# joyecnu/STTODE

Measured on AMD Instinct MI355X. Metric: predicted-trajectories/sec (20-sample best-of-K), higher is better.
Workload: dtype f32

## Files before the change

### profiles/exp_chain_stamps.py

```python
import ctypes, os, sys
import numpy as np, torch
ROOT = os.path.dirname(os.path.dirname(os.path.abspath(__file__)))
sys.path.insert(0, ROOT); sys.path.insert(0, os.path.join(ROOT, 'tests'))
from helpers import make_args
from sttode_amd import STTODENet, capi, scenes
from sttode_amd.weights import make_weights, to_torch_state_dict
dev = torch.device('cuda:0')
m = STTODENet(make_args('eth', 8, 12), dev).eval()
m.load_state_dict(to_torch_state_dict(make_weights(1234)), strict=True)
L = capi.lib()
for S in [int(a) for a in sys.argv[1:]] or [128]:
    sb = scenes.make_scene_batch(range(S), 'eth')
    m.set_scene_batch(sb.past, sb.future, sb.scene_ptr)
    m.native().set_chain(1)
    for _ in range(3):
        m.inference(None)
    ngroups = (sb.n_agents * 20 + 127) // 128
    nwg = max(512, ngroups + (sb.n_agents + 15) // 16)
    dbg = torch.zeros(nwg * 4 * 16, dtype=torch.int64, device=dev)
    L.sttode_chain_debug_buffer.argtypes = [ctypes.c_void_p]
    L.sttode_chain_debug_buffer(dbg.data_ptr())
    m.inference(None)
    torch.cuda.synchronize()
    L.sttode_chain_debug_buffer(None)
    d = dbg.cpu().numpy().reshape(nwg, 4, 8, 2)
    valid = d[:, :, 0, 0] > 0
    cyc = d[..., 0].astype(np.float64); ns = d[..., 1].astype(np.float64) * 10.0
    names = ['mlp0x', 'mlp0y', 'gru', 'mlp1']
    print(f'scenes {S}: {ngroups} groups, {int(valid.sum())} stamped group passes')
    for k in range(4):
        dc = (cyc[:, :, k + 1] - cyc[:, :, k])[valid]; dn = (ns[:, :, k + 1] - ns[:, :, k])[valid]
        print(f'  {names[k]:6s} cycles median {np.median(dc):10.0f} min {dc.min():10.0f} max {dc.max():10.0f} | us median {np.median(dn) / 1e3:8.1f}  -> clock {np.median(dc) / np.median(dn):.2f} GHz')
    tot = (ns[:, :, 4] - ns[:, :, 0])[valid]
    t0 = ns[:, 0, 0][valid[:, 0]]
    print(f'  group total us median {np.median(tot) / 1e3:.1f} min {tot.min() / 1e3:.1f} max {tot.max() / 1e3:.1f}; first-group start spread {(t0.max() - t0.min()) / 1e3:.1f} us; '
          f'kernel span {(ns[:, :, 4][valid].max() - t0.min()) / 1e3:.1f} us')
    b3 = os.environ.get('STTODE_BF16X3', '0') not in ('', '0')
    per_tile = 12 * 32 if b3 else 16 * 64
    ideal = {'mlp0x': 152 * per_tile, 'mlp0y': 152 * per_tile, 'gru': 8 * 37 * per_tile, 'mlp1': 200 * per_tile}
    print('  MFMA-only cycles per phase (' + ('bf16x3' if b3 else 'f32') + '):', ideal)
```

### sttode_amd/csrc/chain.hpp

```cpp
#pragma once
#include <hip/hip_runtime.h>

typedef float f32x4 __attribute__((ext_vector_type(4)));

#define STT_WAVE 64
#define STT_FENCE() asm volatile("" ::: "memory")

__device__ __forceinline__ f32x4 mfma_k16(f32x4 acc, const f32x4 w, const f32x4 b) {
    acc = __builtin_amdgcn_mfma_f32_16x16x4f32(w[0], b[0], acc, 0, 0, 0);
    acc = __builtin_amdgcn_mfma_f32_16x16x4f32(w[1], b[1], acc, 0, 0, 0);
    acc = __builtin_amdgcn_mfma_f32_16x16x4f32(w[2], b[2], acc, 0, 0, 0);
    acc = __builtin_amdgcn_mfma_f32_16x16x4f32(w[3], b[3], acc, 0, 0, 0);
    return acc;
}

__device__ __forceinline__ f32x4 ld4(const float* p) { return *reinterpret_cast<const f32x4*>(p); }
__device__ __forceinline__ void st4(float* p, const f32x4 v) { *reinterpret_cast<f32x4*>(p) = v; }

__device__ __forceinline__ f32x4 relu4(f32x4 v) {
    v[0] = fmaxf(v[0], 0.f); v[1] = fmaxf(v[1], 0.f); v[2] = fmaxf(v[2], 0.f); v[3] = fmaxf(v[3], 0.f);
    return v;
}

__device__ __forceinline__ float sigmoidf_(float x) {
// ... 15 lines not shown

__device__ __forceinline__ void layernorm64(f32x4 (&x)[4], const float* __restrict__ gamma, const float* __restrict__ beta, int q) {
    float s = 0.f;
#pragma unroll
    for (int T = 0; T < 4; ++T) s += (x[T][0] + x[T][1]) + (x[T][2] + x[T][3]);
    const float mean = colsum_q(s) * (1.0f / 64.0f);
    float v = 0.f;
#pragma unroll
    for (int T = 0; T < 4; ++T)
#pragma unroll
        for (int r = 0; r < 4; ++r) { const float d = x[T][r] - mean; v += d * d; }
    const float rstd = 1.0f / sqrtf(colsum_q(v) * (1.0f / 64.0f) + 1e-5f);
#pragma unroll
    for (int T = 0; T < 4; ++T) {
        const f32x4 g = ld4(gamma + 16 * T + 4 * q), b = ld4(beta + 16 * T + 4 * q);
#pragma unroll
        for (int r = 0; r < 4; ++r) x[T][r] = (x[T][r] - mean) * rstd * g[r] + b[r];
    }
}

__device__ __forceinline__ void lds_barrier() { asm volatile("s_waitcnt lgkmcnt(0)\n\ts_barrier" ::: "memory"); }

__device__ __forceinline__ unsigned lds_addr(const void* p) {
    return (unsigned)(size_t)(const __attribute__((address_space(3))) void*)p;
}
__device__ __forceinline__ void glds16_asm(const void* gsrc, unsigned lds_dst) {
    unsigned keep;
    asm volatile("s_mov_b32 %0, m0\n\ts_mov_b32 m0, %2\n\ts_nop 0\n\tglobal_load_lds_dwordx4 %1, off\n\ts_mov_b32 m0, %0"
                 : "=&s"(keep) : "v"(gsrc), "s"(lds_dst) : "memory");
}
template <int OFS>
__device__ __forceinline__ void glds16_sv(const void* sbase, unsigned voff, unsigned lds_dst) {
    static_assert(OFS >= -4096 && OFS <= 4095, "global_load_lds_dwordx4: the immediate offset is 13-bit signed");
    unsigned keep;
    asm volatile("s_mov_b32 %0, m0\n\ts_mov_b32 m0, %3\n\ts_nop 0\n\tglobal_load_lds_dwordx4 %1, %2 offset:%4\n\ts_mov_b32 m0, %0"
                 : "=&s"(keep) : "v"(voff), "s"(sbase), "s"(lds_dst - (unsigned)OFS), "i"(OFS) : "memory");
}
```

### sttode_amd/csrc/chain32.hip

```cpp
#include "chain.hpp"
#include "latency_bodies.hpp"
#include "frontend_body.hpp"
#include "api_util.hpp"
#include "../../include/sttode_hip.h"
#include <cstdlib>
#include <cstddef>

#ifdef C32_DIAG_TRACE
__shared__ long long g_tr_ph[4];
#define C32_TRACE_BEGIN() long long _tr_t0 = 0, _tr_c0 = 0; if (threadIdx.x == 0 && A.dbg) { _tr_t0 = __builtin_amdgcn_s_memrealtime(); _tr_c0 = __builtin_amdgcn_s_memtime(); }
#define C32_TRACE_END(kind) do { if (threadIdx.x == 0 && A.dbg) { \
        const long long _t1 = __builtin_amdgcn_s_memrealtime(); unsigned _hw, _xcc; \
        asm volatile("s_getreg_b32 %0, hwreg(HW_REG_HW_ID)" : "=s"(_hw)); asm volatile("s_getreg_b32 %0, hwreg(HW_REG_XCC_ID)" : "=s"(_xcc)); \
        const unsigned long long _r = atomicAdd((unsigned long long*)A.dbg, 1ull); if ((long long)_r >= A.dbg[1]) break;  \
        long long* _p = A.dbg + 8 + _r * 12; _p[0] = A.trace_tag; _p[1] = blockIdx.x; _p[2] = (kind); _p[3] = _tr_t0; _p[4] = _t1; _p[5] = _hw; _p[6] = _xcc; \
        _p[8] = g_tr_ph[0]; _p[9] = g_tr_ph[1]; _p[10] = g_tr_ph[2]; _p[7] = __builtin_amdgcn_s_memtime() - _tr_c0; _p[11] = g_tr_ph[3]; } } while (0)
#define C32_TRACE_PHASE(i) do { if (threadIdx.x == 0) g_tr_ph[i] = __builtin_amdgcn_s_memrealtime(); } while (0)
#else
#define C32_TRACE_PHASE(i) do { } while (0)
#define C32_TRACE_BEGIN() do { } while (0)
#define C32_TRACE_END(kind) do { } while (0)
#endif

#include "role_body.hpp"
// ... 49 lines not shown
    int xcd_map;
    RoleArgs R;
    Role32Args R32;
};

template <int NY> struct C32Const {
    static constexpr int b2x = 0, b3x = 256, b2y = 288, b3y = 544, gb = 544 + 32 * NY, cb = gb + 384, b2m = cb + 32,
                         b3m = b2m + 256, total = b3m + 32 * NY;
};

__device__ __forceinline__ f32x16 splat16(float v) {
    f32x16 r;
#pragma unroll
    for (int e = 0; e < 16; ++e) r[e] = v;
    return r;
}
__device__ __forceinline__ f32x16 relu16(f32x16 v) {
#pragma unroll
    for (int e = 0; e < 16; ++e) v[e] = fmaxf(v[e], 0.f);
    return v;
}
__device__ __forceinline__ f32x16 ldrows(const float* p, int h) {
    f32x16 r;
#pragma unroll
    for (int a = 0; a < 4; ++a) {
        const f32x4 v = ld4(p + 8 * a + 4 * h);
        r[4 * a + 0] = v[0]; r[4 * a + 1] = v[1]; r[4 * a + 2] = v[2]; r[4 * a + 3] = v[3];
    }
    return r;
}

typedef const __attribute__((address_space(4))) int KProg;

template <int BUF, bool GEN>
struct ChainStreamT {
    static constexpr int kBuf = BUF;
    const char* pool; KProg* prog; f32x4* ring;
    unsigned ring_addr, loff;
    int len, p, par, lane, wave;
    int2 nxt_v;
    int cnt;
    __device__ __forceinline__ int2 entry(int q) const { return make_int2(prog[2 * q], prog[2 * q + 1]); }
    __device__ __forceinline__ void dma(int2 ev, int buf) {
        const char* src = pool + (size_t)ev.x * (GEN ? 16 : C32_TILE * 16) + wave * 1024;
        const int pieces = GEN ? ev.y : 4 * ev.y;
        const unsigned dst = __builtin_amdgcn_readfirstlane(ring_addr + (unsigned)buf * (BUF * 16) + (unsigned)wave * 1024);
#ifndef C32_DIAG_NODMA
#pragma unroll
        for (int i = 0; i < (BUF / 64 + 3) / 4; ++i)
            if (4 * i + wave < pieces) glds16_sv<0>(src + i * 4096, loff, dst + i * 4096);
#endif
    }
    __device__ __forceinline__ void init(const f32x4* pool_, const int2* prog_, int len_, f32x4* ring_) {
        pool = reinterpret_cast<const char*>(pool_); prog = (KProg*)prog_; len = len_; ring = ring_;
        ring_addr = lds_addr(ring_);
        lane = threadIdx.x & 63;
        loff = (unsigned)lane * 16;
        wave = __builtin_amdgcn_readfirstlane(threadIdx.x >> 6);
        p = 0; par = 0;
        const int2 e0 = entry(0);
        cnt = e0.y;
        dma(e0, 0);
        nxt_v = entry(1 % len);
    }
    __device__ __forceinline__ void begin() {
        __builtin_amdgcn_sched_barrier(0);
        cnt = nxt_v.y;
        dma(nxt_v, par ^ 1);
        int q = p + 2;
        q = q >= len ? q - len : q;
        nxt_v = entry(q);
        __builtin_amdgcn_sched_barrier(0);
    }
    __device__ __forceinline__ const f32x4* cur() const { return ring + par * BUF + lane; }
    __device__ __forceinline__ void end() {
        __builtin_amdgcn_sched_barrier(0);
#ifndef C32_DIAG_NOBARRIER
        asm volatile("s_waitcnt vmcnt(0)" ::: "memory");
        __syncthreads();
#endif
        p = p + 1 >= len ? 0 : p + 1;
        par ^= 1;
        __builtin_amdgcn_sched_barrier(0);
    }
};
typedef ChainStreamT<C32_CMAX * C32_TILE, false> ChainStream;

__device__ __forceinline__ void tile_mma(f32x16& acc, const f32x4* __restrict__ t, const f32x16& B) {
#pragma unroll
    for (int g = 0; g < 4; ++g) {
        const f32x4 a = t[g * 64];
#pragma unroll
        for (int r = 0; r < 4; ++r) acc = __builtin_amdgcn_mfma_f32_32x32x2f32(a[r], B[4 * g + r], acc, 0, 0, 0);
    }
}

__device__ __forceinline__ void gather_rows(const void* base, unsigned voff, unsigned slot_addr) {
    glds16_sv<0>(base, voff, slot_addr);
    glds16_sv<32>(base, voff, slot_addr + 1024);
    glds16_sv<64>(base, voff, slot_addr + 2048);
    glds16_sv<96>(base, voff, slot_addr + 3072);
}
__device__ __forceinline__ unsigned row_off(int row, int width, int h) { return (unsigned)row * (unsigned)(width * 4) + (unsigned)h * 16; }

struct Frag { f32x4 a[4]; };
__device__ __forceinline__ void ldfrag(Frag& f, const f32x4* __restrict__ t) {
#pragma unroll
    for (int g = 0; g < 4; ++g) f.a[g] = t[g * 64];
}
__device__ __forceinline__ void tile_mma2(f32x16& acc, const Frag& cur, const f32x16& B, Frag& nxt, const f32x4* __restrict__ tn) {
#pragma unroll
    for (int g = 0; g < 4; ++g) {
        if (g == 2 && tn) {
            ldfrag(nxt, tn);
            __builtin_amdgcn_sched_barrier(0);
        }
#pragma unroll
        for (int r = 0; r < 4; ++r) acc = __builtin_amdgcn_mfma_f32_32x32x2f32(cur.a[g][r], B[4 * g + r], acc, 0, 0, 0);
    }
}

template <int KH, class ST>
__device__ __forceinline__ void mlp_l12(ST& st, const f32x4* slot, const f32x4* zslot, const f32x16* Bh, const float* tab, unsigned aoff,
                                        const float* tab_next, unsigned aoff_next, f32x16 (&acc2)[8], int lane) {
    const unsigned slot_addr = __builtin_amdgcn_readfirstlane(lds_addr(slot));
    constexpr int KT1 = 1 + KH;
    static_assert((KT1 + 8) % 3 == 0, "hidden tile must be a whole number of chunks");
#pragma unroll
    for (int R = 0; R < 8; ++R) acc2[R] = splat16(0.f);
#pragma unroll 1
    for (int ht = 0; ht < 16; ++ht) {
        f32x16 h1, zb;
#pragma unroll
        for (int a = 0; a < 4; ++a) {
            const f32x4 v = slot[a * 64 + lane];
            h1[4 * a + 0] = v[0]; h1[4 * a + 1] = v[1]; h1[4 * a + 2] = v[2]; h1[4 * a + 3] = v[3];
        }
#pragma unroll
        for (int a = 0; a < 4; ++a) {
            const f32x4 v = zslot[a * 64 + lane];
            zb[4 * a + 0] = v[0]; zb[4 * a + 1] = v[1]; zb[4 * a + 2] = v[2]; zb[4 * a + 3] = v[3];
        }
        asm volatile("s_waitcnt lgkmcnt(0)" ::: "memory");
        __builtin_amdgcn_sched_barrier(0);
        const bool nl = ht + 1 < 16;
        const void* nb = nl ? (const void*)(reinterpret_cast<const char*>(tab) + 128 * (ht + 1)) : (const void*)tab_next;
        const unsigned no = nl ? aoff : aoff_next;
        Frag fr[2];
#pragma unroll
        for (int i = 0; i < KT1 + 8; ++i) {
            if (i % 3 == 0) {
                if (i > 0) st.end();
                ldfrag(fr[i & 1], st.cur());
                st.begin();
                if (i == 0) {
#ifndef C32_DIAG_NOGATHER
                    gather_rows(nb, no, slot_addr);
#endif
                    __builtin_amdgcn_sched_barrier(0);
                }
            }
            const f32x4* tn = (i % 3 < 2) ? st.cur() + (i % 3 + 1) * C32_TILE : nullptr;
            if (i == 0) {
                tile_mma2(h1, fr[i & 1], zb, fr[(i + 1) & 1], tn);
            } else if (i < KT1) {
                tile_mma2(h1, fr[i & 1], Bh[i - 1], fr[(i + 1) & 1], tn);
            } else {
                if (i == KT1) h1 = relu16(h1);
                tile_mma2(acc2[i - KT1], fr[i & 1], h1, fr[(i + 1) & 1], tn);
            }
        }
        st.end();
    }
}

template <int NO, class ST>
__device__ __forceinline__ void mlp_l3(ST& st, f32x16 (&acc2)[8], const float* __restrict__ b2, const float* __restrict__ b3,
                                       f32x16 (&out)[NO], int h) {
#pragma unroll
    for (int R = 0; R < 8; ++R) {
        STT_FENCE();
        const f32x16 b = ldrows(b2 + 32 * R, h);
        acc2[R] = relu16(acc2[R] + b);
        asm volatile("" : "+v"(acc2[R]));
    }
    STT_FENCE();
#pragma unroll
    for (int o = 0; o < NO; ++o) out[o] = ldrows(b3 + 32 * o, h);
    Frag fr[2];
#pragma unroll
    for (int i = 0; i < 8 * NO; ++i) {
        if (i % 3 == 0) {
            if (i > 0) st.end();
            ldfrag(fr[i & 1], st.cur());
            st.begin();
        }
        const f32x4* tn = (i % 3 < 2 && i + 1 < 8 * NO) ? st.cur() + (i % 3 + 1) * C32_TILE : nullptr;
        tile_mma2(out[i / 8], fr[i & 1], acc2[i % 8], fr[(i + 1) & 1], tn);
    }
    st.end();
}

typedef __bf16 bf16x8 __attribute__((ext_vector_type(8)));
typedef __bf16 bf16x2 __attribute__((ext_vector_type(2)));
typedef float f32x2v __attribute__((ext_vector_type(2)));
typedef unsigned u32x4v __attribute__((ext_vector_type(4)));
#define C32_TILE_B3 384
#define C32_BUF_B3 (C32_CMAX * C32_TILE_B3)
struct B3 { bf16x8 p[3][2]; };
__device__ __forceinline__ float bf_lo(unsigned u) { return __uint_as_float(u << 16); }
__device__ __forceinline__ float bf_hi(unsigned u) { return __uint_as_float(u & 0xffff0000u); }
__device__ __forceinline__ void split3(const f32x16& x, B3& o) {
#pragma unroll
    for (int kb = 0; kb < 2; ++kb) {
        unsigned hi[4], mi[4], lo[4];
#pragma unroll
        for (int q = 0; q < 4; ++q) {
            const float x0 = x[8 * kb + 2 * q], x1 = x[8 * kb + 2 * q + 1];
            const f32x2v v = {x0, x1};
            hi[q] = __builtin_bit_cast(unsigned, __builtin_convertvector(v, bf16x2));
            const float r0 = x0 - bf_lo(hi[q]), r1 = x1 - bf_hi(hi[q]);
            const f32x2v rv = {r0, r1};
            mi[q] = __builtin_bit_cast(unsigned, __builtin_convertvector(rv, bf16x2));
            const f32x2v qv = {r0 - bf_lo(mi[q]), r1 - bf_hi(mi[q])};
            lo[q] = __builtin_bit_cast(unsigned, __builtin_convertvector(qv, bf16x2));
        }
        const u32x4v H = {hi[0], hi[1], hi[2], hi[3]}, M = {mi[0], mi[1], mi[2], mi[3]}, L = {lo[0], lo[1], lo[2], lo[3]};
        o.p[0][kb] = __builtin_bit_cast(bf16x8, H);
        o.p[1][kb] = __builtin_bit_cast(bf16x8, M);
        o.p[2][kb] = __builtin_bit_cast(bf16x8, L);
    }
// ... 178 lines not shown
            tile_mma_b3n(az, st.cur() + T, hB[2]);
#pragma unroll
            for (int r = 0; r < 16; ++r) az[r] = C32_SIG(az[r]);
            STT_FENCE();
            f32x16 an = ldrows(gb + 3 * 96 + 32 * j, h);
            tile_mma_b3n(an, st.cur() + 2 * T, hB[0]);
            st.end(); st.begin();
            tile_mma_b3n(an, st.cur(), hB[1]);
            tile_mma_b3n(an, st.cur() + T, hB[2]);
            {
                const f32x16 bi = ldrows(gb + 2 * 96 + 32 * j, h);
#pragma unroll
                for (int r = 0; r < 16; ++r) an[r] = fmaf(ar[r], an[r], bi[r]);
            }
            STT_FENCE();
            tile_mma_b3n(an, st.cur() + 2 * T, eB);
            st.end();
            const f32x16 hp = b3_to_f32(hB[j]);
#pragma unroll
            for (int r = 0; r < 16; ++r) {
                const float ng = C32_TANH(an[r]);
                hn[j][r] = fmaf(az[r], hp[r] - ng, ng);
            }
        }
#pragma unroll
        for (int j = 0; j < 3; ++j) {
            hs[j] = hn[j];
            split3(hn[j], hB[j]);
        }
    }
}

template <bool ZS, class ST>
__device__ __forceinline__ f32x16 gru32_conv(ST& st, const float* cb, const f32x16& d, int t, int Tp, int h) {
    f32x16 e = ldrows(cb, h);
    Frag fa, fb;
    if (ZS) {
        const int k0 = 2 * t - 2, k1 = 2 * t + 3;
        const int g0 = (k0 > 0 ? k0 : 0) >> 3, g1 = (k1 < 2 * Tp - 1 ? k1 : 2 * Tp - 1) >> 3;
        const f32x4* tc = st.cur();
#pragma unroll
        for (int g = 0; g < 4; ++g)
            if (g >= g0 && g <= g1) fa.a[g] = tc[g * 64];
        st.begin();
#pragma unroll
        for (int g = 0; g < 4; ++g)
            if (g >= g0 && g <= g1)
#pragma unroll
                for (int r = 0; r < 4; ++r) e = __builtin_amdgcn_mfma_f32_32x32x2f32(fa.a[g][r], d[4 * g + r], e, 0, 0, 0);
    } else {
        ldfrag(fa, st.cur());
        st.begin();
        tile_mma2(e, fa, d, fb, nullptr);
    }
    e = relu16(e);
    st.end();
    return e;
}

template <bool ZS, class ST>
__device__ __forceinline__ void gru32_steps(ST& st, const float* gb, const float* cb, const f32x16& d, f32x16 (&hs)[3], int Tp, int h) {
    if (ZS) {
        const f32x16 e = gru32_conv<ZS>(st, cb, d, 0, Tp, h);
        Frag fa, fb;
#pragma unroll
        for (int j = 0; j < 3; ++j) {
            STT_FENCE();
            f32x16 ar = ldrows(gb + 0 * 96 + 32 * j, h);
            ldfrag(fa, st.cur()); st.begin();
            tile_mma2(ar, fa, e, fb, nullptr);
            st.end(); ldfrag(fa, st.cur() + 1 * C32_TILE); st.begin();
#pragma unroll
            for (int r = 0; r < 16; ++r) ar[r] = C32_SIG(ar[r]);
            STT_FENCE();
            f32x16 az = ldrows(gb + 1 * 96 + 32 * j, h);
            tile_mma2(az, fa, e, fb, nullptr);
            st.end(); st.begin();
#pragma unroll
            for (int r = 0; r < 16; ++r) az[r] = C32_SIG(az[r]);
            STT_FENCE();
            f32x16 an = ldrows(gb + 3 * 96 + 32 * j, h);
            {
                const f32x16 bi = ldrows(gb + 2 * 96 + 32 * j, h);
#pragma unroll
                for (int r = 0; r < 16; ++r) an[r] = fmaf(ar[r], an[r], bi[r]);
            }
            st.end(); ldfrag(fa, st.cur() + 2 * C32_TILE); st.begin();
            STT_FENCE();
            tile_mma2(an, fa, e, fb, nullptr);
            st.end();
#pragma unroll
            for (int r = 0; r < 16; ++r) {
                const float ng = C32_TANH(an[r]);
                hs[j][r] = fmaf(az[r], 0.f - ng, ng);
            }
        }
    }
#pragma unroll 1
    for (int t = ZS ? 1 : 0; t < Tp; ++t) {
        const f32x16 e = gru32_conv<ZS>(st, cb, d, t, Tp, h);
        Frag fa, fb;
        f32x16 hn[3];
#pragma unroll
        for (int j = 0; j < 3; ++j) {
            STT_FENCE();
            f32x16 ar = ldrows(gb + 0 * 96 + 32 * j, h);
            ldfrag(fa, st.cur()); st.begin();
            tile_mma2(ar, fa, e, fb, st.cur() + 1 * C32_TILE);
            tile_mma2(ar, fb, hs[0], fa, st.cur() + 2 * C32_TILE);
            tile_mma2(ar, fa, hs[1], fb, nullptr);
            st.end(); ldfrag(fa, st.cur()); st.begin();
            tile_mma2(ar, fa, hs[2], fb, st.cur() + 1 * C32_TILE);
#pragma unroll
            for (int r = 0; r < 16; ++r) ar[r] = C32_SIG(ar[r]);
            STT_FENCE();
            f32x16 az = ldrows(gb + 1 * 96 + 32 * j, h);
            tile_mma2(az, fb, e, fa, st.cur() + 2 * C32_TILE);
            tile_mma2(az, fa, hs[0], fb, nullptr);
            st.end(); ldfrag(fa, st.cur()); st.begin();
            tile_mma2(az, fa, hs[1], fb, st.cur() + 1 * C32_TILE);
            tile_mma2(az, fb, hs[2], fa, st.cur() + 2 * C32_TILE);
#pragma unroll
            for (int r = 0; r < 16; ++r) az[r] = C32_SIG(az[r]);
            STT_FENCE();
            f32x16 an = ldrows(gb + 3 * 96 + 32 * j, h);
            tile_mma2(an, fa, hs[0], fb, nullptr);
            st.end(); ldfrag(fa, st.cur()); st.begin();
            tile_mma2(an, fa, hs[1], fb, st.cur() + 1 * C32_TILE);
            tile_mma2(an, fb, hs[2], fa, st.cur() + 2 * C32_TILE);
            {
                const f32x16 bi = ldrows(gb + 2 * 96 + 32 * j, h);
#pragma unroll
                for (int r = 0; r < 16; ++r) an[r] = fmaf(ar[r], an[r], bi[r]);
            }
            STT_FENCE();
            tile_mma2(an, fa, e, fb, nullptr);
            st.end();
#pragma unroll
            for (int r = 0; r < 16; ++r) {
                const float ng = C32_TANH(an[r]);
                hn[j][r] = fmaf(az[r], hs[j][r] - ng, ng);
            }
        }
#pragma unroll
        for (int j = 0; j < 3; ++j) hs[j] = hn[j];
    }

}

#include "role32.hpp"

__device__ __forceinline__ int opaque(int v) { asm volatile("" : "+v"(v)); return v; }

#ifdef C32_DIAG_STAMPS
#define C32_STAMP(k) do { if (threadIdx.x == 0 && A.dbg && gi < 4) { A.dbg[((size_t)blockIdx.x * 4 + gi) * 16 + 2 * (k)] = __builtin_amdgcn_s_memtime(); \
                                                                    A.dbg[((size_t)blockIdx.x * 4 + gi) * 16 + 2 * (k) + 1] = __builtin_amdgcn_s_memrealtime(); } } while (0)
#else
#define C32_STAMP(k) do { } while (0)
#endif

__host__ __device__ __forceinline__ int fused_block_of(long b, long T, long G, long K, long lead) {
    auto roles_upto = [&](long x) { const long c = (8 * (x + lead + 1) + K - 1) / K; return c < T ? c : T; };
    long lo = -1, hi = G - 1;
    while (lo < hi) {
        const long mid = (lo + hi + 1) >> 1;
        if (mid + roles_upto(mid) <= b) lo = mid; else hi = mid - 1;
    }
    if (lo >= 0 && lo + roles_upto(lo) == b) return (int)lo;
    return -1 - (int)(b - (lo + 1));
}

__host__ __device__ __forceinline__ int xcd_group(int b, int G) {
    const int x = b & 7, i = b >> 3, q = G >> 3, r = G & 7;
    return x * q + (x < r ? x : r) + i;
}

template <int NY, int FUSE, bool B3M, bool ZS>
__global__ __launch_bounds__(256, 2) void traj_chain_kernel(ChainArgs A) {
    typedef ChainStreamT<B3M ? C32_BUF_B3 : C32_CMAX * C32_TILE, B3M> Stream;
    extern __shared__ __attribute__((aligned(16))) char smem[];
    f32x4* ring = reinterpret_cast<f32x4*>(smem);
    f32x4* slots = ring + 2 * Stream::kBuf;
    f32x4* zslots = slots + 4 * C32_SLOT;
    float* cst = reinterpret_cast<float*>(zslots + 4 * C32_SLOT);
    int* sq = reinterpret_cast<int*>(cst + C32Const<NY>::total);
    typedef C32Const<NY> CO;

    const int lane = threadIdx.x & 63, c = lane & 31, h = lane >> 5;
    const int wave = __builtin_amdgcn_readfirstlane(threadIdx.x >> 6);
    const f32x4* slot = slots + wave * C32_SLOT;
    const f32x4* zslot = zslots + wave * C32_SLOT;
    const unsigned slot_addr = __builtin_amdgcn_readfirstlane(lds_addr(slot));
    const unsigned zslot_addr = __builtin_amdgcn_readfirstlane(lds_addr(zslot));
    const int ngroups = (A.ncols + 127) >> 7;

    C32_TRACE_BEGIN();
    if (FUSE == 2 && (int)blockIdx.x < A.R32.nwg) {
        role32_body<ZS>(*(KRole32Args*)((const __attribute__((address_space(4))) char*)__builtin_amdgcn_kernarg_segment_ptr() + offsetof(ChainArgs, R32)),
                    blockIdx.x, smem);
        C32_TRACE_END(1);
        return;
    }
    if (FUSE == 1 && A.R.split && (int)blockIdx.x < 5 * A.R.ntiles) {
        split_role(A.R, (A.ncols + A.K - 1) / A.K, A.Tp, A.ldx, A.xpad, blockIdx.x, smem);
        C32_TRACE_END(1);
        return;
    }
    int fb = FUSE == 0 ? (int)blockIdx.x : FUSE == 2 ? (int)blockIdx.x - A.R32.nwg : A.R.split ? (int)blockIdx.x - 5 * A.R.ntiles
                                                : fused_block_of(blockIdx.x, A.R.ntiles, ngroups, A.K, A.R.lead);
    if (FUSE && A.xcd_map && fb >= 0) fb = xcd_group(fb, ngroups);
    if (FUSE == 1 && fb < 0) {
        agent_role(A.R, (A.ncols + A.K - 1) / A.K, A.Tp, A.ldx, A.xpad, -1 - fb, smem);
// ... 29 lines not shown
    auto col_of = [&](int gg) { int col = gg * 128 + wave * 32 + c; return col < A.ncols ? col : A.ncols - 1; };
    {
        const int c0 = col_of(g);
        gather_rows(A.A0x, row_off(c0 / A.K, 512, h), slot_addr);
        gather_rows(A.z, row_off(c0, 32, h), zslot_addr);
    }
    asm volatile("s_waitcnt vmcnt(0)" ::: "memory");
    __syncthreads();

    int gi = 0;
    (void)gi;
    while (true) {
        C32_STAMP(0);
        const int col = g * 128 + wave * 32 + c;
        int colc = col < A.ncols ? col : A.ncols - 1;
        int agent = colc / A.K;
        const bool live = col < A.ncols;
        __syncthreads();
        if (threadIdx.x == 0)
            sq[1] = (FUSE == 2 && A.persistent && ngroups > A.nworkers) ? A.nworkers + atomicAdd(A.counter, 1)
                    : (FUSE == 0 && A.persistent) ? atomicAdd(A.counter, 1) : ngroups;

        f32x16 acc2[8];
        f32x16 d;
        {
            agent = opaque(agent);
            f32x16 xo[1];
            const unsigned ao = row_off(agent, 512, h);
            if (B3M) {
                mlp_l12_b3<0, true>(st, slot, zslot, nullptr, A.A0x, ao, A.A0y, ao, acc2, lane);
                mlp_l3_b3<1>(st, acc2, cst + CO::b2x, cst + CO::b3x, xo, h);
            } else {
                mlp_l12<0>(st, slot, zslot, nullptr, A.A0x, ao, A.A0y, ao, acc2, lane);
                mlp_l3<1>(st, acc2, cst + CO::b2x, cst + CO::b3x, xo, h);
            }
            agent = opaque(agent);
            const float* xp = A.xpad + (size_t)agent * A.ldx;
#pragma unroll
            for (int a = 0; a < 4; ++a) {
                f32x4 v = splat4(0.f);
                if (8 * a + 4 * h < A.ldx) v = ld4(xp + 8 * a + 4 * h);
#pragma unroll
                for (int b = 0; b < 4; ++b) d[4 * a + b] = v[b] - xo[0][4 * a + b];
            }
        }
        STT_FENCE();
        C32_STAMP(1);
        {
            agent = opaque(agent);
            f32x16 yo[NY];
            const unsigned ao = row_off(agent, 512, h);
            if (B3M) {
                mlp_l12_b3<0, true>(st, slot, zslot, nullptr, A.A0y, ao, A.A1y, ao, acc2, lane);
                mlp_l3_b3<NY>(st, acc2, cst + CO::b2y, cst + CO::b3y, yo, h);
            } else {
                mlp_l12<0>(st, slot, zslot, nullptr, A.A0y, ao, A.A1y, ao, acc2, lane);
                mlp_l3<NY>(st, acc2, cst + CO::b2y, cst + CO::b3y, yo, h);
            }
            if (live) {
                float* prow = A.park + (size_t)opaque(col) * A.Tf2;
#pragma unroll
                for (int o = 0; o < NY; ++o)
#pragma unroll
                    for (int a = 0; a < 4; ++a) {
                        const int row0 = 32 * o + 8 * a + 4 * h;
                        float* p = prow + row0;
                        if (row0 + 3 < A.Tf2 && (A.Tf2 & 3) == 0) {
                            f32x4 v = {yo[o][4 * a], yo[o][4 * a + 1], yo[o][4 * a + 2], yo[o][4 * a + 3]};
                            st4(p, v);
                        } else {
#pragma unroll
                            for (int b = 0; b < 4; ++b)
                                if (row0 + b < A.Tf2) p[b] = yo[o][4 * a + b];
                        }
                    }
            }
        }
        STT_FENCE();
        C32_STAMP(2);
        f32x16 hs[3];
        {
#pragma unroll
            for (int j = 0; j < 3; ++j) hs[j] = splat16(0.f);
            if (B3M) gru32_steps_b3(st, cst + CO::gb, cst + CO::cb, d, hs, A.Tp, h);
            else gru32_steps<ZS>(st, cst + CO::gb, cst + CO::cb, d, hs, A.Tp, h);
        }
        STT_FENCE();
        C32_STAMP(3);
        const int gnext = sq[1];
        {
            agent = opaque(agent);
            const int cnx = col_of(gnext < ngroups ? gnext : g);
            const unsigned ao = row_off(agent, 512, h), an = row_off(cnx / A.K, 512, h);
            if (B3M) mlp_l12_b3<3, false>(st, slot, zslot, hs, A.A1y, ao, A.A0x, an, acc2, lane);
            else mlp_l12<3>(st, slot, zslot, hs, A.A1y, ao, A.A0x, an, acc2, lane);
            gather_rows(A.z, row_off(opaque(cnx), 32, h), zslot_addr);
            f32x16 yo[NY];
            if (B3M) mlp_l3_b3<NY>(st, acc2, cst + CO::b2m, cst + CO::b3m, yo, h);
            else mlp_l3<NY>(st, acc2, cst + CO::b2m, cst + CO::b3m, yo, h);
            {
                agent = opaque(agent);
                const float cx = A.cur[2 * agent], cy = A.cur[2 * agent + 1];
                const float ox = A.orig[2 * agent], oy = A.orig[2 * agent + 1];
                const bool vec = (A.Tf2 & 3) == 0;
                const float* yrow = A.park + (size_t)opaque(colc) * A.Tf2;
                float* prow = A.pred + (size_t)opaque(col) * A.Tf2;
                const float* grow = FUSE == 2 && A.m_gt ? A.m_gt + (size_t)agent * A.Tf2 : nullptr;
                float dd[NY][4][2];
#pragma unroll
                for (int o = 0; o < NY; ++o)
#pragma unroll
                    for (int a = 0; a < 4; ++a) {
                        const int row0 = 32 * o + 8 * a + 4 * h;
                        const bool whole = vec && row0 + 3 < A.Tf2;
                        f32x4 y0 = splat4(0.f);
                        if (whole) y0 = ld4(yrow + row0);
                        else {
#pragma unroll
                            for (int b = 0; b < 4; ++b)
                                if (row0 + b < A.Tf2) y0[b] = yrow[row0 + b];
                        }
                        f32x4 v;
                        v[0] = ((y0[0] + yo[o][4 * a + 0]) + cx) + ox;
                        v[1] = ((y0[1] + yo[o][4 * a + 1]) + cy) + oy;
                        v[2] = ((y0[2] + yo[o][4 * a + 2]) + cx) + ox;
                        v[3] = ((y0[3] + yo[o][4 * a + 3]) + cy) + oy;
                        if (live) {
                            if (whole) st4(prow + row0, v);
                            else {
#pragma unroll
                                for (int b = 0; b < 4; ++b)
                                    if (row0 + b < A.Tf2) prow[row0 + b] = v[b];
// ... 1 lines not shown
                        }
                        dd[o][a][0] = dd[o][a][1] = 0.f;
                        if (FUSE == 2 && grow) {
                            if (row0 < A.Tf2) { const float2 g = *reinterpret_cast<const float2*>(grow + row0); dd[o][a][0] = bok_dist(v[0], v[1], g.x, g.y, A.m_scale); }
                            if (row0 + 2 < A.Tf2) { const float2 g = *reinterpret_cast<const float2*>(grow + row0 + 2); dd[o][a][1] = bok_dist(v[2], v[3], g.x, g.y, A.m_scale); }
                        }
                    }
                if (FUSE == 2 && grow) {
                    const int Tf = A.Tf2 >> 1;
                    float acc = 0.f, fdl = -1.f;
#pragma unroll
                    for (int o = 0; o < NY; ++o)
#pragma unroll
                        for (int a = 0; a < 4; ++a) {
                            const int t0 = (32 * o + 8 * a + 4 * h) >> 1;
                            float mine = acc;
                            if (h == 0) { if (t0 < Tf) mine += dd[o][a][0]; if (t0 + 1 < Tf) mine += dd[o][a][1]; }
                            float mine1 = __shfl(mine, c, 64);
                            if (h == 1) { if (t0 < Tf) mine1 += dd[o][a][0]; if (t0 + 1 < Tf) mine1 += dd[o][a][1]; }
                            acc = __shfl(mine1, c + 32, 64);
                            if (t0 == Tf - 1) fdl = dd[o][a][0];
                            if (t0 + 1 == Tf - 1) fdl = dd[o][a][1];
                        }
                    fdl = fmaxf(fdl, __shfl_xor(fdl, 32, 64));
                    const float adev = acc / (float)Tf;
                    if (live && h == 0) {
                        atomicMin(reinterpret_cast<unsigned*>(A.m_ade) + agent, __float_as_uint(adev));
                        atomicMin(reinterpret_cast<unsigned*>(A.m_fde) + agent, __float_as_uint(fdl));
                    }
                }
            }
        }
        C32_STAMP(4);
        ++gi;
        g = gnext;
        if (g >= ngroups) break;
    }
    C32_TRACE_END(0);
}

struct Gru32Args {
    const float* xin; int ldx;
    const f32x4* pool; const int2* prog; int prog_len;
    const float* consts;
    float* state;
    int ncols, Tp;
};
template <bool ZS>
__global__ __launch_bounds__(256, 2) void gru32_kernel(Gru32Args A) {
    extern __shared__ __attribute__((aligned(16))) char smem[];
    f32x4* ring = reinterpret_cast<f32x4*>(smem);
    float* cst = reinterpret_cast<float*>(ring + C32_RING);
    const int lane = threadIdx.x & 63, c = lane & 31, h = lane >> 5;
    const int wave = __builtin_amdgcn_readfirstlane(threadIdx.x >> 6);
    for (int i = threadIdx.x; i < 416; i += blockDim.x) cst[i] = A.consts[i];
    __syncthreads();
    ChainStream st;
    st.init(A.pool, A.prog, A.prog_len, ring);
    const int col = blockIdx.x * 128 + wave * 32 + c;
    const int colc = col < A.ncols ? col : A.ncols - 1;
    f32x16 d;
    {
        const float* xp = A.xin + (size_t)colc * A.ldx;
#pragma unroll
        for (int a = 0; a < 4; ++a) {
            f32x4 v = splat4(0.f);
// ... 324 lines not shown
```

### sttode_amd/csrc/role32.hpp

```cpp
#pragma once

struct R32C {
    static constexpr int bc = 0, wlast = 64, bi = 128, bg = 192, ln1w = 256, ln1b = 320, l1b = 384, l2b = 1408, ln2w = 1472, ln2b = 1536,
                         gb = 1600, cb = 1984, b1x = 2016, b1y = 2528, b11 = 3040, total = 3552;
};

typedef const __attribute__((address_space(4))) Role32Args KRole32Args;

template <class ST> struct TileFeed {
    ST& st; int t, cnt; bool pre;
    Frag cur, nxt;
    __device__ __forceinline__ explicit TileFeed(ST& s) : st(s), t(0), cnt(0), pre(false) {}
    __device__ __forceinline__ void open() {
        cnt = st.cnt;
        t = 0;
        ldfrag(cur, st.cur());
        st.begin();
        pre = false;
    }
    __device__ __forceinline__ void mma(f32x16& acc, const f32x16& B) {
        if (t == cnt) { st.end(); open(); }
        else if (pre) cur = nxt;
        const f32x4* tn = t + 1 < cnt ? st.cur() + (t + 1) * C32_TILE : nullptr;
        tile_mma2(acc, cur, B, nxt, tn);
        pre = tn != nullptr;
        ++t;
    }
    __device__ __forceinline__ void close() { st.end(); }
};

__device__ __forceinline__ float halfsum32(float v) { return v + __shfl_xor(v, 32, 64); }

__device__ __forceinline__ void layernorm64_c32(f32x16 (&x)[2], const float* gamma, const float* beta, int h) {
    float s = 0.f;
#pragma unroll
    for (int j = 0; j < 2; ++j)
#pragma unroll
        for (int r = 0; r < 16; r += 4) s += (x[j][r] + x[j][r + 1]) + (x[j][r + 2] + x[j][r + 3]);
    const float mean = halfsum32(s) * (1.0f / 64.0f);
    float v = 0.f;
#pragma unroll
    for (int j = 0; j < 2; ++j)
#pragma unroll
        for (int r = 0; r < 16; ++r) { const float dd = x[j][r] - mean; v += dd * dd; }
    const float rstd = 1.0f / sqrtf(halfsum32(v) * (1.0f / 64.0f) + 1e-5f);
#pragma unroll
    for (int j = 0; j < 2; ++j) {
        const f32x16 g = ldrows(gamma + 32 * j, h), b = ldrows(beta + 32 * j, h);
#pragma unroll
        for (int r = 0; r < 16; ++r) x[j][r] = (x[j][r] - mean) * rstd * g[r] + b[r];
    }
}

__device__ __forceinline__ void strows(float* p, const f32x16& v, int h) {
#pragma unroll
    for (int a = 0; a < 4; ++a) {
        const f32x4 w = {v[4 * a], v[4 * a + 1], v[4 * a + 2], v[4 * a + 3]};
        st4(p + 8 * a + 4 * h, w);
    }
}

// ... 68 lines not shown
    const int lane = threadIdx.x & 63, c = lane & 31, h = lane >> 5;
    const int wave = __builtin_amdgcn_readfirstlane(threadIdx.x >> 6);
    if (R.prio > 0) __builtin_amdgcn_s_setprio(3);
    if (wg == 0 && threadIdx.x == 0) *R.counter = 0;
    if (R.m_ade && threadIdx.x < 128 && wg * 128 + (int)threadIdx.x < R.n) {
        R.m_ade[wg * 128 + threadIdx.x] = INFINITY;
        R.m_fde[wg * 128 + threadIdx.x] = INFINITY;
    }
    if (R.past) frontend32(R, wg);
    if (R.zgen) latents32(R.zgen, R.zkey0, R.zkey1, wg, R.n, R.K);
    if (R.past) {
        __builtin_amdgcn_fence(__ATOMIC_RELEASE, "workgroup");
        __syncthreads();
        __builtin_amdgcn_fence(__ATOMIC_ACQUIRE, "workgroup");
    }
    for (int i = threadIdx.x; i < R32C::total; i += blockDim.x) cst[i] = R.consts[i];
    __syncthreads();
    ChainStream st;
    st.init(R.pool, R.prog, R.prog_len, ring);
    const int col = wg * 128 + wave * 32 + c;
    const bool live = col < R.n;
    const int colc = live ? col : R.n - 1;
    f32x16 d;
    {
        const float* xp = R.xpad + (size_t)colc * R.ldx;
#pragma unroll
        for (int a = 0; a < 4; ++a) {
            f32x4 v = splat4(0.f);
            if (8 * a + 4 * h < R.ldx) v = ld4(xp + 8 * a + 4 * h);
#pragma unroll
            for (int b = 0; b < 4; ++b) d[4 * a + b] = v[b];
        }
    }
    asm volatile("s_waitcnt vmcnt(0)" ::: "memory");
    __syncthreads();
    f32x16 hs[3];
#pragma unroll
    for (int j = 0; j < 3; ++j) hs[j] = splat16(0.f);
    gru32_steps<ZS>(st, cst + R32C::gb, cst + R32C::cb, d, hs, R.Tp, h);
    if (live) {
#pragma unroll
        for (int j = 0; j < 3; ++j) strows(R.state0 + (size_t)col * 96 + 32 * j, hs[j], h);
    }
    STT_FENCE();
    TileFeed<ChainStream> fd(st);
    fd.open();
    f32x16 G[2], S[2];
    if (R.attn == nullptr) {
        f32x16 X[2];
        const float* ep = R.enc_in + (size_t)colc * (4 * R.Tp);
#pragma unroll
        for (int kt = 0; kt < 2; ++kt)
#pragma unroll
            for (int a = 0; a < 4; ++a) {
                f32x4 v = splat4(0.f);
                if (32 * kt + 8 * a + 4 * h < 4 * R.Tp) v = ld4(ep + 32 * kt + 8 * a + 4 * h);
#pragma unroll
                for (int b = 0; b < 4; ++b) X[kt][4 * a + b] = v[b];
            }
        const float lastf = R.last[colc] ? 1.0f : 0.0f;
#pragma unroll
        for (int j = 0; j < 2; ++j) {
            const f32x16 b = ldrows(cst + R32C::bc + 32 * j, h), wl = ldrows(cst + R32C::wlast + 32 * j, h);
#pragma unroll
            for (int r = 0; r < 16; ++r) G[j][r] = fmaf(wl[r], lastf, b[r]);
            fd.mma(G[j], X[0]);
            if (R.kte > 1) fd.mma(G[j], X[1]);
        }
        S[0] = G[0]; S[1] = G[1];
    } else {
#pragma unroll
        for (int j = 0; j < 2; ++j) {
// ... 117 lines not shown
```

Before: 85.66 million.

## Prefetch weight-stream program entries mid-tile and precompute DMA addresses before barrier

```diff
diff --git a/profiles/exp_chain_stamps.py b/profiles/exp_chain_stamps.py
--- a/profiles/exp_chain_stamps.py
+++ b/profiles/exp_chain_stamps.py
@@ -35,6 +35,13 @@
     t0 = ns[:, 0, 0][valid[:, 0]]
     print(f'  group total us median {np.median(tot) / 1e3:.1f} min {tot.min() / 1e3:.1f} max {tot.max() / 1e3:.1f}; first-group start spread {(t0.max() - t0.min()) / 1e3:.1f} us; '
           f'kernel span {(ns[:, :, 4][valid].max() - t0.min()) / 1e3:.1f} us')
+    gc, gn, cal = cyc[:, :, 5][valid], d[:, :, 5, 1].astype(np.float64)[valid], cyc[:, :, 6][valid]
+    if gn.max() > 0:
+        per = gc / gn - cal
+        tot_c = (cyc[:, :, 4] - cyc[:, :, 0])[valid]
+        print(f'  chunk step, barrier -> first MFMA ready: {np.median(gn):.0f} steps per group; cycles per step median {np.median(per):.1f} '
+              f'(p10 {np.percentile(per, 10):.1f}, p90 {np.percentile(per, 90):.1f}; empty stamp pair {np.median(cal):.0f} taken off); '
+              f'per group median {np.median(per * gn):.0f} = {100 * np.median(per * gn / tot_c):.2f} % of the group\'s {np.median(tot_c):.0f} cycles')
     b3 = os.environ.get('STTODE_BF16X3', '0') not in ('', '0')
     per_tile = 12 * 32 if b3 else 16 * 64
     ideal = {'mlp0x': 152 * per_tile, 'mlp0y': 152 * per_tile, 'gru': 8 * 37 * per_tile, 'mlp1': 200 * per_tile}
diff --git a/sttode_amd/csrc/chain.hpp b/sttode_amd/csrc/chain.hpp
--- a/sttode_amd/csrc/chain.hpp
+++ b/sttode_amd/csrc/chain.hpp
@@ -71,7 +71,11 @@
 template <int OFS>
 __device__ __forceinline__ void glds16_sv(const void* sbase, unsigned voff, unsigned lds_dst) {
     static_assert(OFS >= -4096 && OFS <= 4095, "global_load_lds_dwordx4: the immediate offset is 13-bit signed");
-    unsigned keep;
-    asm volatile("s_mov_b32 %0, m0\n\ts_mov_b32 m0, %3\n\ts_nop 0\n\tglobal_load_lds_dwordx4 %1, %2 offset:%4\n\ts_mov_b32 m0, %0"
-                 : "=&s"(keep) : "v"(voff), "s"(sbase), "s"(lds_dst - (unsigned)OFS), "i"(OFS) : "memory");
+    asm volatile("s_mov_b32 m0, %2\n\ts_nop 0\n\tglobal_load_lds_dwordx4 %0, %1 offset:%3"
+                 : : "v"(voff), "s"(sbase), "s"(lds_dst - (unsigned)OFS), "i"(OFS) : "memory");
 }
+template <int OFS>
+__device__ __forceinline__ void glds16_m0(const void* sbase, unsigned voff) {
+    static_assert(OFS >= -4096 && OFS <= 4095, "global_load_lds_dwordx4: the immediate offset is 13-bit signed");
+    asm volatile("global_load_lds_dwordx4 %0, %1 offset:%2" : : "v"(voff), "s"(sbase), "i"(OFS) : "memory");
+}
diff --git a/sttode_amd/csrc/chain32.hip b/sttode_amd/csrc/chain32.hip
--- a/sttode_amd/csrc/chain32.hip
+++ b/sttode_amd/csrc/chain32.hip
@@ -105,55 +105,114 @@
 
 typedef const __attribute__((address_space(4))) int KProg;
 
-template <int BUF, bool GEN>
+template <int BUF, bool GEN, bool DYN = false>
 struct ChainStreamT {
     static constexpr int kBuf = BUF;
+    static constexpr int kPieces = (BUF / 64 + 3) / 4, kPairs = (kPieces + 1) / 2;
     const char* pool; KProg* prog; f32x4* ring;
     unsigned ring_addr, loff;
-    int len, p, par, lane, wave;
-    int2 nxt_v;
+    unsigned qoff, qend;
+    int par, lane, wave;
+    int2 ld_v, ld_w;
+    bool fetched;
     int cnt;
-    __device__ __forceinline__ int2 entry(int q) const { return make_int2(prog[2 * q], prog[2 * q + 1]); }
-    __device__ __forceinline__ void dma(int2 ev, int buf) {
-        const char* src = pool + (size_t)ev.x * (GEN ? 16 : C32_TILE * 16) + wave * 1024;
-        const int pieces = GEN ? ev.y : 4 * ev.y;
-        const unsigned dst = __builtin_amdgcn_readfirstlane(ring_addr + (unsigned)buf * (BUF * 16) + (unsigned)wave * 1024);
+    const char* nsrc[kPairs]; unsigned nm0[kPairs]; int ncnt, npc;
+#ifdef C32_DIAG_STAMPS
+    long long t_bar, gap_cyc, gap_n, gap_cal;
+#endif
+    __device__ __forceinline__ int2 entry_at(unsigned off) const {
+        const KProg* e = reinterpret_cast<const KProg*>(reinterpret_cast<const __attribute__((address_space(4))) char*>(prog) + off);
+        return make_int2(e[0], e[1]);
+    }
+    __device__ __forceinline__ unsigned next_off(unsigned off) const { return off + 8 >= qend ? 0u : off + 8; }
+    __device__ __forceinline__ void stage(int2 ev, int buf) {
+        ncnt = __builtin_amdgcn_readfirstlane(ev.y);
+        npc = GEN ? (ncnt - wave + 3) >> 2 : ncnt;
+        const size_t src = (size_t)(unsigned)__builtin_amdgcn_readfirstlane(ev.x) * (GEN ? 16u : C32_TILE * 16u) + (unsigned)wave * 1024u;
+        const unsigned dst = __builtin_amdgcn_readfirstlane(ring_addr + (unsigned)buf * (BUF * 16) + (unsigned)wave * 1024u);
+#pragma unroll
+        for (int k = 0; k < kPairs; ++k) {
+            nsrc[k] = pool + (src + 4096u * (2 * k + 1));
+            nm0[k] = dst + 4096u * (2 * k + 1);
+            asm volatile("" : "+s"(nsrc[k]), "+s"(nm0[k]));
+        }
+        asm volatile("" : "+s"(npc));
+    }
+    __device__ __forceinline__ void issue(int N) {
 #ifndef C32_DIAG_NODMA
 #pragma unroll
-        for (int i = 0; i < (BUF / 64 + 3) / 4; ++i)
-            if (4 * i + wave < pieces) glds16_sv<0>(src + i * 4096, loff, dst + i * 4096);
+        for (int k = 0; k < kPairs; ++k) {
+            if (N > 0 ? 2 * k < N : 2 * k < npc) {
+                glds16_sv<-4096>(nsrc[k], loff, nm0[k] - 4096u);
+                if (2 * k + 1 < kPieces && (N > 0 ? 2 * k + 1 < N : 2 * k + 1 < npc)) glds16_m0<0>(nsrc[k], loff);
+            }
+        }
 #endif
     }
     __device__ __forceinline__ void init(const f32x4* pool_, const int2* prog_, int len_, f32x4* ring_) {
-        pool = reinterpret_cast<const char*>(pool_); prog = (KProg*)prog_; len = len_; ring = ring_;
-        ring_addr = lds_addr(ring_);
+        pool = reinterpret_cast<const char*>(pool_); prog = (KProg*)prog_; ring = ring_;
+        ring_addr = __builtin_amdgcn_readfirstlane(lds_addr(ring_));
         lane = threadIdx.x & 63;
         loff = (unsigned)lane * 16;
         wave = __builtin_amdgcn_readfirstlane(threadIdx.x >> 6);
-        p = 0; par = 0;
-        const int2 e0 = entry(0);
+        par = 0;
+        qend = (unsigned)len_ * 8u;
+        const int2 e0 = entry_at(0);
+        stage(e0, 0);
+        issue(0);
         cnt = e0.y;
-        dma(e0, 0);
-        nxt_v = entry(1 % len);
-    }
-    __device__ __forceinline__ void begin() {
+        qoff = next_off(0);
+        stage(entry_at(qoff), 1);
+        qoff = next_off(qoff);
+        fetched = false;
+#ifdef C32_DIAG_STAMPS
+        gap_cyc = 0; gap_n = 0;
+        const long long c0 = __builtin_amdgcn_s_memtime();
+        asm volatile("s_waitcnt lgkmcnt(0)" ::: "memory");
+        gap_cal = __builtin_amdgcn_s_memtime() - c0;
+        t_bar = 0;
+#endif
+    }
+    __device__ __forceinline__ void fetch() { ld_v = entry_at(qoff); qoff = next_off(qoff); fetched = true; }
+    __device__ __forceinline__ void fetch_more() { ld_w = entry_at(qoff); qoff = next_off(qoff); }
+    __device__ __forceinline__ void take_prefetched() { ld_v = ld_w; fetched = true; }
+    __device__ __forceinline__ void stamp_gap() {
+#ifdef C32_DIAG_STAMPS
+        asm volatile("s_waitcnt lgkmcnt(0)" ::: "memory");
+        const long long c1 = __builtin_amdgcn_s_memtime();
+        asm volatile("s_waitcnt lgkmcnt(0)" ::: "memory");
+        if (t_bar) { gap_cyc += c1 - t_bar; ++gap_n; }
+#endif
+    }
+    __device__ __forceinline__ void begin(int N = 0) {
         __builtin_amdgcn_sched_barrier(0);
-        cnt = nxt_v.y;
-        dma(nxt_v, par ^ 1);
-        int q = p + 2;
-        q = q >= len ? q - len : q;
-        nxt_v = entry(q);
+#ifdef C32_DIAG_CHECK
+        if (!GEN && N > 0 && ncnt != N) __builtin_trap();
+#endif
+        cnt = ncnt;
+        issue(GEN || DYN ? 0 : N);
+        stamp_gap();
         __builtin_amdgcn_sched_barrier(0);
     }
     __device__ __forceinline__ const f32x4* cur() const { return ring + par * BUF + lane; }
-    __device__ __forceinline__ void end() {
+    __device__ __forceinline__ void end(bool has_entry = false) {
+        __builtin_amdgcn_sched_barrier(0);
+#ifdef C32_DIAG_CHECK
+        if (has_entry && !fetched) __builtin_trap();
+#endif
+        if (!has_entry && !fetched) fetch();
+        stage(ld_v, par);
         __builtin_amdgcn_sched_barrier(0);
 #ifndef C32_DIAG_NOBARRIER
         asm volatile("s_waitcnt vmcnt(0)" ::: "memory");
         __syncthreads();
 #endif
-        p = p + 1 >= len ? 0 : p + 1;
+#ifdef C32_DIAG_STAMPS
+        t_bar = __builtin_amdgcn_s_memtime();
+        asm volatile("s_waitcnt lgkmcnt(0)" ::: "memory");
+#endif
         par ^= 1;
+        fetched = false;
         __builtin_amdgcn_sched_barrier(0);
     }
 };
@@ -186,6 +245,22 @@
     for (int g = 0; g < 4; ++g) {
         if (g == 2 && tn) {
             ldfrag(nxt, tn);
+            __builtin_amdgcn_sched_barrier(0);
+        }
+#pragma unroll
+        for (int r = 0; r < 4; ++r) acc = __builtin_amdgcn_mfma_f32_32x32x2f32(cur.a[g][r], B[4 * g + r], acc, 0, 0, 0);
+    }
+}
+
+template <class ST>
+__device__ __forceinline__ void tile_mma2f(ST& st, f32x16& acc, const Frag& cur, const f32x16& B, Frag& nxt, const f32x4* __restrict__ tn, int nf = 1) {
+#pragma unroll
+    for (int g = 0; g < 4; ++g) {
+        if (g == 2) {
+            __builtin_amdgcn_sched_barrier(0);
+            if (nf >= 1) st.fetch();
+            if (nf >= 2) st.fetch_more();
+            if (tn) ldfrag(nxt, tn);
             __builtin_amdgcn_sched_barrier(0);
         }
 #pragma unroll
@@ -225,7 +300,7 @@
             if (i % 3 == 0) {
                 if (i > 0) st.end();
                 ldfrag(fr[i & 1], st.cur());
-                st.begin();
+                st.begin(3);
                 if (i == 0) {
 #ifndef C32_DIAG_NOGATHER
                     gather_rows(nb, no, slot_addr);
@@ -235,19 +310,21 @@
             }
             const f32x4* tn = (i % 3 < 2) ? st.cur() + (i % 3 + 1) * C32_TILE : nullptr;
             if (i == 0) {
-                tile_mma2(h1, fr[i & 1], zb, fr[(i + 1) & 1], tn);
+                tile_mma2f(st, h1, fr[i & 1], zb, fr[(i + 1) & 1], tn);
             } else if (i < KT1) {
-                tile_mma2(h1, fr[i & 1], Bh[i - 1], fr[(i + 1) & 1], tn);
+                if (i % 3 == 0) tile_mma2f(st, h1, fr[i & 1], Bh[i - 1], fr[(i + 1) & 1], tn);
+                else tile_mma2(h1, fr[i & 1], Bh[i - 1], fr[(i + 1) & 1], tn);
             } else {
                 if (i == KT1) h1 = relu16(h1);
-                tile_mma2(acc2[i - KT1], fr[i & 1], h1, fr[(i + 1) & 1], tn);
+                if (i % 3 == 0) tile_mma2f(st, acc2[i - KT1], fr[i & 1], h1, fr[(i + 1) & 1], tn);
+                else tile_mma2(acc2[i - KT1], fr[i & 1], h1, fr[(i + 1) & 1], tn);
             }
         }
         st.end();
     }
 }
 
-template <int NO, class ST>
+template <int NO, int NEXT = 0, class ST>
 __device__ __forceinline__ void mlp_l3(ST& st, f32x16 (&acc2)[8], const float* __restrict__ b2, const float* __restrict__ b3,
                                        f32x16 (&out)[NO], int h) {
 #pragma unroll
@@ -266,10 +343,12 @@
         if (i % 3 == 0) {
             if (i > 0) st.end();
             ldfrag(fr[i & 1], st.cur());
-            st.begin();
+            const int left = 8 * NO - (i + 3);
+            st.begin(left >= 3 ? 3 : left > 0 ? left : NEXT);
         }
         const f32x4* tn = (i % 3 < 2 && i + 1 < 8 * NO) ? st.cur() + (i % 3 + 1) * C32_TILE : nullptr;
-        tile_mma2(out[i / 8], fr[i & 1], acc2[i % 8], fr[(i + 1) & 1], tn);
+        if (i % 3 == 0) tile_mma2f(st, out[i / 8], fr[i & 1], acc2[i % 8], fr[(i + 1) & 1], tn);
+        else tile_mma2(out[i / 8], fr[i & 1], acc2[i % 8], fr[(i + 1) & 1], tn);
     }
     st.end();
 }
@@ -514,7 +593,7 @@
 }
 
 template <bool ZS, class ST>
-__device__ __forceinline__ f32x16 gru32_conv(ST& st, const float* cb, const f32x16& d, int t, int Tp, int h) {
+__device__ __forceinline__ f32x16 gru32_conv(ST& st, const float* cb, const f32x16& d, int t, int Tp, int h, bool pre) {
     f32x16 e = ldrows(cb, h);
     Frag fa, fb;
     if (ZS) {
@@ -524,16 +603,20 @@
 #pragma unroll
         for (int g = 0; g < 4; ++g)
             if (g >= g0 && g <= g1) fa.a[g] = tc[g * 64];
-        st.begin();
+        st.begin(3);
 #pragma unroll
         for (int g = 0; g < 4; ++g)
             if (g >= g0 && g <= g1)
 #pragma unroll
                 for (int r = 0; r < 4; ++r) e = __builtin_amdgcn_mfma_f32_32x32x2f32(fa.a[g][r], d[4 * g + r], e, 0, 0, 0);
+        __builtin_amdgcn_sched_barrier(0);
+        if (pre) st.take_prefetched();
+        else st.fetch();
     } else {
         ldfrag(fa, st.cur());
-        st.begin();
-        tile_mma2(e, fa, d, fb, nullptr);
+        st.begin(3);
+        tile_mma2f(st, e, fa, d, fb, nullptr, pre ? 0 : 1);
+        if (pre) st.take_prefetched();
     }
     e = relu16(e);
     st.end();
@@ -543,21 +626,22 @@
 template <bool ZS, class ST>
 __device__ __forceinline__ void gru32_steps(ST& st, const float* gb, const float* cb, const f32x16& d, f32x16 (&hs)[3], int Tp, int h) {
     if (ZS) {
-        const f32x16 e = gru32_conv<ZS>(st, cb, d, 0, Tp, h);
+        const f32x16 e = gru32_conv<ZS>(st, cb, d, 0, Tp, h, false);
         Frag fa, fb;
 #pragma unroll
         for (int j = 0; j < 3; ++j) {
             STT_FENCE();
             f32x16 ar = ldrows(gb + 0 * 96 + 32 * j, h);
-            ldfrag(fa, st.cur()); st.begin();
-            tile_mma2(ar, fa, e, fb, nullptr);
-            st.end(); ldfrag(fa, st.cur() + 1 * C32_TILE); st.begin();
+            ldfrag(fa, st.cur()); st.begin(3);
+            tile_mma2f(st, ar, fa, e, fb, nullptr);
+            st.end(); ldfrag(fa, st.cur() + 1 * C32_TILE); st.begin(3);
 #pragma unroll
             for (int r = 0; r < 16; ++r) ar[r] = C32_SIG(ar[r]);
             STT_FENCE();
             f32x16 az = ldrows(gb + 1 * 96 + 32 * j, h);
-            tile_mma2(az, fa, e, fb, nullptr);
-            st.end(); st.begin();
+            tile_mma2f(st, az, fa, e, fb, nullptr, 2);
+            st.end(); st.begin(3);
+            st.take_prefetched();
 #pragma unroll
             for (int r = 0; r < 16; ++r) az[r] = C32_SIG(az[r]);
             STT_FENCE();
@@ -567,9 +651,10 @@
 #pragma unroll
                 for (int r = 0; r < 16; ++r) an[r] = fmaf(ar[r], an[r], bi[r]);
             }
-            st.end(); ldfrag(fa, st.cur() + 2 * C32_TILE); st.begin();
+            st.end(); ldfrag(fa, st.cur() + 2 * C32_TILE);
+            if (j < 2) st.begin(3); else st.begin();
             STT_FENCE();
-            tile_mma2(an, fa, e, fb, nullptr);
+            tile_mma2f(st, an, fa, e, fb, nullptr, (j == 2 && 1 < Tp) ? 2 : 1);
             st.end();
 #pragma unroll
             for (int r = 0; r < 16; ++r) {
@@ -580,35 +665,36 @@
     }
 #pragma unroll 1
     for (int t = ZS ? 1 : 0; t < Tp; ++t) {
-        const f32x16 e = gru32_conv<ZS>(st, cb, d, t, Tp, h);
+        const f32x16 e = gru32_conv<ZS>(st, cb, d, t, Tp, h, ZS);
         Frag fa, fb;
         f32x16 hn[3];
 #pragma unroll
         for (int j = 0; j < 3; ++j) {
             STT_FENCE();
             f32x16 ar = ldrows(gb + 0 * 96 + 32 * j, h);
-            ldfrag(fa, st.cur()); st.begin();
-            tile_mma2(ar, fa, e, fb, st.cur() + 1 * C32_TILE);
+            ldfrag(fa, st.cur()); st.begin(3);
+            tile_mma2f(st, ar, fa, e, fb, st.cur() + 1 * C32_TILE);
             tile_mma2(ar, fb, hs[0], fa, st.cur() + 2 * C32_TILE);
             tile_mma2(ar, fa, hs[1], fb, nullptr);
-            st.end(); ldfrag(fa, st.cur()); st.begin();
-            tile_mma2(ar, fa, hs[2], fb, st.cur() + 1 * C32_TILE);
+            st.end(); ldfrag(fa, st.cur()); st.begin(3);
+            tile_mma2f(st, ar, fa, hs[2], fb, st.cur() + 1 * C32_TILE);
 #pragma unroll
             for (int r = 0; r < 16; ++r) ar[r] = C32_SIG(ar[r]);
             STT_FENCE();
             f32x16 az = ldrows(gb + 1 * 96 + 32 * j, h);
             tile_mma2(az, fb, e, fa, st.cur() + 2 * C32_TILE);
             tile_mma2(az, fa, hs[0], fb, nullptr);
-            st.end(); ldfrag(fa, st.cur()); st.begin();
-            tile_mma2(az, fa, hs[1], fb, st.cur() + 1 * C32_TILE);
+            st.end(); ldfrag(fa, st.cur()); st.begin(3);
+            tile_mma2f(st, az, fa, hs[1], fb, st.cur() + 1 * C32_TILE);
             tile_mma2(az, fb, hs[2], fa, st.cur() + 2 * C32_TILE);
 #pragma unroll
             for (int r = 0; r < 16; ++r) az[r] = C32_SIG(az[r]);
             STT_FENCE();
             f32x16 an = ldrows(gb + 3 * 96 + 32 * j, h);
             tile_mma2(an, fa, hs[0], fb, nullptr);
-            st.end(); ldfrag(fa, st.cur()); st.begin();
-            tile_mma2(an, fa, hs[1], fb, st.cur() + 1 * C32_TILE);
+            st.end(); ldfrag(fa, st.cur());
+            if (j < 2) st.begin(3); else st.begin();
+            tile_mma2f(st, an, fa, hs[1], fb, st.cur() + 1 * C32_TILE, (ZS && j == 2 && t + 1 < Tp) ? 2 : 1);
             tile_mma2(an, fb, hs[2], fa, st.cur() + 2 * C32_TILE);
             {
                 const f32x16 bi = ldrows(gb + 2 * 96 + 32 * j, h);
@@ -659,7 +745,8 @@
 
 template <int NY, int FUSE, bool B3M, bool ZS>
 __global__ __launch_bounds__(256, 2) void traj_chain_kernel(ChainArgs A) {
-    typedef ChainStreamT<B3M ? C32_BUF_B3 : C32_CMAX * C32_TILE, B3M> Stream;
+    constexpr bool kDynCount = !B3M && ((NY == 1 && FUSE == 2 && !ZS) || (NY == 2 && FUSE == 1 && ZS));
+    typedef ChainStreamT<B3M ? C32_BUF_B3 : C32_CMAX * C32_TILE, B3M, kDynCount> Stream;
     extern __shared__ __attribute__((aligned(16))) char smem[];
     f32x4* ring = reinterpret_cast<f32x4*>(smem);
     f32x4* slots = ring + 2 * Stream::kBuf;
@@ -755,7 +842,7 @@
                 mlp_l3_b3<1>(st, acc2, cst + CO::b2x, cst + CO::b3x, xo, h);
             } else {
                 mlp_l12<0>(st, slot, zslot, nullptr, A.A0x, ao, A.A0y, ao, acc2, lane);
-                mlp_l3<1>(st, acc2, cst + CO::b2x, cst + CO::b3x, xo, h);
+                mlp_l3<1, 3>(st, acc2, cst + CO::b2x, cst + CO::b3x, xo, h);
             }
             agent = opaque(agent);
             const float* xp = A.xpad + (size_t)agent * A.ldx;
@@ -778,7 +865,7 @@
                 mlp_l3_b3<NY>(st, acc2, cst + CO::b2y, cst + CO::b3y, yo, h);
             } else {
                 mlp_l12<0>(st, slot, zslot, nullptr, A.A0y, ao, A.A1y, ao, acc2, lane);
-                mlp_l3<NY>(st, acc2, cst + CO::b2y, cst + CO::b3y, yo, h);
+                mlp_l3<NY, 1>(st, acc2, cst + CO::b2y, cst + CO::b3y, yo, h);
             }
             if (live) {
                 float* prow = A.park + (size_t)opaque(col) * A.Tf2;
@@ -820,7 +907,7 @@
             gather_rows(A.z, row_off(opaque(cnx), 32, h), zslot_addr);
             f32x16 yo[NY];
             if (B3M) mlp_l3_b3<NY>(st, acc2, cst + CO::b2m, cst + CO::b3m, yo, h);
-            else mlp_l3<NY>(st, acc2, cst + CO::b2m, cst + CO::b3m, yo, h);
+            else mlp_l3<NY, 3>(st, acc2, cst + CO::b2m, cst + CO::b3m, yo, h);
             {
                 agent = opaque(agent);
                 const float cx = A.cur[2 * agent], cy = A.cur[2 * agent + 1];
@@ -888,6 +975,13 @@
             }
         }
         C32_STAMP(4);
+#ifdef C32_DIAG_STAMPS
+        if (threadIdx.x == 0 && A.dbg && gi < 4) {
+            long long* o = A.dbg + ((size_t)blockIdx.x * 4 + gi) * 16 + 10;
+            o[0] = st.gap_cyc; o[1] = st.gap_n; o[2] = st.gap_cal;
+        }
+        st.gap_cyc = 0; st.gap_n = 0;
+#endif
         ++gi;
         g = gnext;
         if (g >= ngroups) break;
diff --git a/sttode_amd/csrc/role32.hpp b/sttode_amd/csrc/role32.hpp
--- a/sttode_amd/csrc/role32.hpp
+++ b/sttode_amd/csrc/role32.hpp
@@ -19,14 +19,14 @@
         pre = false;
     }
     __device__ __forceinline__ void mma(f32x16& acc, const f32x16& B) {
-        if (t == cnt) { st.end(); open(); }
+        if (t == cnt) { st.end(true); open(); }
         else if (pre) cur = nxt;
         const f32x4* tn = t + 1 < cnt ? st.cur() + (t + 1) * C32_TILE : nullptr;
-        tile_mma2(acc, cur, B, nxt, tn);
+        tile_mma2f(st, acc, cur, B, nxt, tn, t == 0 ? 1 : 0);
         pre = tn != nullptr;
         ++t;
     }
-    __device__ __forceinline__ void close() { st.end(); }
+    __device__ __forceinline__ void close() { st.end(true); }
 };
 
 __device__ __forceinline__ float halfsum32(float v) { return v + __shfl_xor(v, 32, 64); }
@@ -161,12 +161,14 @@
             for (int b = 0; b < 4; ++b) d[4 * a + b] = v[b];
         }
     }
+    int Tp = R.Tp;
+    asm volatile("" : "+s"(Tp));
     asm volatile("s_waitcnt vmcnt(0)" ::: "memory");
     __syncthreads();
     f32x16 hs[3];
 #pragma unroll
     for (int j = 0; j < 3; ++j) hs[j] = splat16(0.f);
-    gru32_steps<ZS>(st, cst + R32C::gb, cst + R32C::cb, d, hs, R.Tp, h);
+    gru32_steps<ZS>(st, cst + R32C::gb, cst + R32C::cb, d, hs, Tp, h);
     if (live) {
 #pragma unroll
         for (int j = 0; j < 3; ++j) strows(R.state0 + (size_t)col * 96 + 32 * j, hs[j], h);
```

Result: faster. 86.70 million (median of 6 runs) (+1.2%).
